# slp-rl/slamkit

Hardware: NVIDIA H100
Metric: speech-tokens/sec (SLAM seq=1024) (higher is better)
Workload: dtype bf16

## Files before the change

### include/slamkit_b200.h

```cpp
#ifndef SLAMKIT_B200_H
#define SLAMKIT_B200_H

#include <stdint.h>

#ifdef __cplusplus
extern "C" {
#endif

const char* sk_last_error(void);
int sk_version(void);
int sk_device_sm_count(void);
int sk_device_cc(void);

int sk_gemm_bf16(int M, int N, int K, const void* A, int lda, int a_mn, const void* B, int ldb, int b_mn, void* C,
                 int ldc, int out_f32, const void* bias, const void* residual, int ldr, int round_before_res, int act,
                 int force_bn, void* stream);

int sk_gemm_bf16_splitk(int M, int N, int K, const void* A, int lda, int a_mn, const void* B, int ldb, int b_mn, void* C,
                        int ldc, int accumulate, void* splitk_ws, int64_t splitk_ws_bytes, void* stream);

int sk_gemm_bf16_ws(int M, int N, int K, const void* A, int lda, int a_mn, const void* B, int ldb, int b_mn, void* C,
                    int ldc, int out_f32, const void* bias, const void* residual, int ldr, int round_before_res, int act,
                    int force_bn, void* ws, int64_t ws_bytes, void* stream);
int64_t sk_gemm_ws_bytes(void);
// ... 56 lines not shown
            int n_rot_heads, int head_dim, int inverse, int max_positions, void* stream);
int sk_swiglu_fwd(const void* gu, void* act, int M, int F, void* stream);
int sk_swiglu_bwd(const void* gu, const void* dact, void* dgu, int M, int F, void* stream);
int sk_ce_blocks(int M);
int sk_ce_fwd_bwd(const void* logits, const int64_t* labels, void* dlogits, float* partial, float* row_nll,
                  float* stats, int M, int T, int V, int ldl, float num_items, float dloss, void* stream);

int sk_attn_fwd(const void* q, const void* k, const void* v, void* o, float* lse, int B, int T, int H, int KVH, int ld,
                int ldo, int causal, float scale, void* stream);
int sk_attn_tc_fwd(const void* qkv, void* o, float* lse, int B, int T, int H, int KVH, int ld, int ldo, int causal,
                   float scale, const int32_t* seg_start, void* stream);
int sk_seg_bounds(const int32_t* pos_ids, int32_t* seg_start, int32_t* seg_end, int B, int T, void* stream);
int sk_attn_tc_bwd(const void* qkv, const void* o, const void* d_o, const float* lse, float* delta, float* partial,
                   void* dqkv, int B, int T, int H, int KVH, int ld, int ldo, int ldg, int causal, float scale,
                   const int32_t* seg_start, const int32_t* seg_end, void* stream);
int sk_attn_bwd(const void* q, const void* k, const void* v, const void* o, const void* d_o, const float* lse,
                float* delta, void* dq, void* dk, void* dv, int B, int T, int H, int KVH, int ld, int ldo, int ldg,
                int causal, float scale, void* stream);
int sk_attn_tc_fwd_split(const void* qkv_hi, const void* qkv_lo, void* o_hi, void* o_lo, int B, int T, int H, int ld,
                         int ldo, float scale, void* stream);

int sk_grad_norm(const void* grads, const int64_t* chunk_start, const int32_t* chunk_len, int n_chunks,
                 const int32_t* tensor_chunk_begin, int n_tensors, float* partial, float max_norm, int emulate_bf16,
                 float* stats, void* stream);
int sk_adamw_step(void* params, const void* grads, void* exp_avg, void* exp_avg_sq, int64_t n, float lr, float beta1,
                  float beta2, float eps, float weight_decay, int step, const float* clip_stats, void* stream);

typedef struct SkLmConfig {
  int32_t vocab_size;
  int32_t hidden;
// ... 183 lines not shown
```

### slamkit_b200/csrc/api.cu

```cuda
#include <stdlib.h>
#include "kernels.h"
#include "../../include/slamkit_b200.h"
#include <atomic>
#include <stdarg.h>
#include <stdio.h>
#include <string.h>
#include <vector>

namespace {
thread_local char g_err[1024] = "";
std::atomic<long long> g_launches{0};
}

void sk_set_error(const char* fmt, ...) {
  va_list ap;
  va_start(ap, fmt);
  vsnprintf(g_err, sizeof(g_err), fmt, ap);
  va_end(ap);
}
bool sk_pdl_enabled() {
  static const bool on = [] { const char* e = getenv("SK_PDL"); return e ? atoi(e) != 0 : true; }();
  return on;
}
void sk_count_launch() { g_launches.fetch_add(1, std::memory_order_relaxed); }
// ... 195 lines not shown
int sk_attn_tc_fwd(const void* qkv, void* o, float* lse, int B, int T, int H, int KVH, int ld, int ldo, int causal,
                   float scale, const int32_t* seg_start, void* stream) {
  SK_REQUIRE(qkv && o, "sk_attn_tc_fwd: null argument");
  return sk_attn_tc_fwd_launch(CBF(qkv), BF(o), lse, B, T, H, KVH, ld, ldo, causal, scale, S(stream), seg_start);
}
int sk_seg_bounds(const int32_t* pos_ids, int32_t* seg_start, int32_t* seg_end, int B, int T, void* stream) {
  return sk_seg_bounds_launch(pos_ids, seg_start, seg_end, B, T, S(stream));
}
int sk_attn_tc_bwd(const void* qkv, const void* o, const void* d_o, const float* lse, float* delta, float* partial,
                   void* dqkv, int B, int T, int H, int KVH, int ld, int ldo, int ldg, int causal, float scale,
                   const int32_t* seg_start, const int32_t* seg_end, void* stream) {
  SK_REQUIRE(qkv && o && d_o && lse && delta && dqkv, "sk_attn_tc_bwd: null argument");
  return sk_attn_tc_bwd_launch(CBF(qkv), CBF(o), CBF(d_o), lse, delta, partial, BF(dqkv), B, T, H, KVH, ld, ldo, ldg, causal,
                               scale, S(stream), seg_start, seg_end);
}
int sk_attn_tc_fwd_split(const void* qkv_hi, const void* qkv_lo, void* o_hi, void* o_lo, int B, int T, int H, int ld,
                         int ldo, float scale, void* stream) {
  SK_REQUIRE(qkv_hi && qkv_lo && o_hi && o_lo, "sk_attn_tc_fwd_split: null argument");
  return sk_attn_tc_fwd_split_launch(CBF(qkv_hi), CBF(qkv_lo), BF(o_hi), BF(o_lo), B, T, H, ld, ldo, scale, S(stream));
}
int sk_attn_bwd(const void* q, const void* k, const void* v, const void* o, const void* d_o, const float* lse,
                float* delta, void* dq, void* dk, void* dv, int B, int T, int H, int KVH, int ld, int ldo, int ldg,
                int causal, float scale, void* stream) {
  return sk_attn_bwd_launch(CBF(q), CBF(k), CBF(v), CBF(o), CBF(d_o), lse, delta, BF(dq), BF(dk), BF(dv), B, T, H, KVH,
                            ld, ldo, ldg, causal, scale, S(stream));
}
int sk_grad_norm(const void* grads, const int64_t* chunk_start, const int32_t* chunk_len, int n_chunks,
                 const int32_t* tensor_chunk_begin, int n_tensors, float* partial, float max_norm, int emulate_bf16,
                 float* stats, void* stream) {
  return sk_gradnorm_launch(CBF(grads), reinterpret_cast<const long*>(chunk_start), chunk_len, n_chunks,
// ... 38 lines not shown
```

### slamkit_b200/csrc/attention.cu

```cuda
#include "kernels.h"

namespace {

constexpr int HD = 64;

SK_DEVINL uint32_t tile_addr(uint32_t base, int r, int chunk) { return base + r * 128 + ((chunk ^ (r & 7)) << 4); }
SK_DEVINL uint32_t smem_base_1k(const void* p) { return (smem_u32(p) + 1023u) & ~1023u; }

SK_DEVINL void cp_async16(uint32_t saddr, const void* g, bool pred) {
  const int sz = pred ? 16 : 0;
  asm volatile("cp.async.cg.shared.global [%0], [%1], 16, %2;" ::"r"(saddr), "l"(g), "r"(sz) : "memory");
}
SK_DEVINL void cp_async_commit() { asm volatile("cp.async.commit_group;" ::: "memory"); }
template <int N>
SK_DEVINL void cp_async_wait() {
  asm volatile("cp.async.wait_group %0;" ::"n"(N) : "memory");
}

SK_DEVINL void wgmma_m64n64_rs(float (&d)[32], const uint32_t (&a)[4], uint64_t db) {
  asm volatile(
      "{\n\t.reg .pred p;\n\tsetp.eq.u32 p, 1, 1;\n\t"
      "wgmma.mma_async.sync.aligned.m64n64k16.f32.bf16.bf16 {%0,%1,%2,%3,%4,%5,%6,%7,%8,%9,%10,%11,%12,%13,%14,%15,"
      "%16,%17,%18,%19,%20,%21,%22,%23,%24,%25,%26,%27,%28,%29,%30,%31}, {%32,%33,%34,%35}, %36, p, 1, 1, 1;\n\t}\n"
      : "+f"(d[0]), "+f"(d[1]), "+f"(d[2]), "+f"(d[3]), "+f"(d[4]), "+f"(d[5]), "+f"(d[6]), "+f"(d[7]), "+f"(d[8]),
        "+f"(d[9]), "+f"(d[10]), "+f"(d[11]), "+f"(d[12]), "+f"(d[13]), "+f"(d[14]), "+f"(d[15]), "+f"(d[16]),
        "+f"(d[17]), "+f"(d[18]), "+f"(d[19]), "+f"(d[20]), "+f"(d[21]), "+f"(d[22]), "+f"(d[23]), "+f"(d[24]),
// ... 59 lines not shown
  const uint32_t sV = sK + 2 * 64 * 128;
  const int b = blockIdx.z, h = blockIdx.y;
  const int qt = gridDim.x - 1 - blockIdx.x;
  const int q0 = qt * 128;
  const int warp = threadIdx.x >> 5, lane = threadIdx.x & 31;
  const bf16* qp = q + (size_t)b * T * ld + h * HD;
  const bf16* kp = k + (size_t)b * T * ld + (h / group) * HD;
  const bf16* vp = v + (size_t)b * T * ld + (h / group) * HD;
  const float sl2 = scale * 1.4426950408889634f;

  int n_kv = (T + 63) / 64;
  if (CAUSAL) {
    const int last = min(T - 1, q0 + 127);
    n_kv = last / 64 + 1;
  }
  load_tile<128, 256>(sQ, qp, ld, q0, T);
  load_tile<64, 256>(sK, kp, ld, 0, T);
  load_tile<64, 256>(sV, vp, ld, 0, T);
  cp_async_commit();

  const uint32_t sQw = sQ + (uint32_t)(warp >> 2) * 8192u;
  float oacc[8][4];
  zero_acc(oacc);
  float m_i[2] = {-INFINITY, -INFINITY}, l_i[2] = {0.f, 0.f};
  const int row_a = q0 + warp * 16 + (lane >> 2);
  int seg_r[2] = {0, 0};
#pragma unroll
  for (int r = 0; r < 2; ++r)
    if (seg_start && row_a + 8 * r < T) seg_r[r] = seg_start[(size_t)b * T + row_a + 8 * r];

  for (int j = 0; j < n_kv; ++j) {
    const int st = j & 1;
    if (j + 1 < n_kv) {
      load_tile<64, 256>(sK + (st ^ 1) * 8192, kp, ld, (j + 1) * 64, T);
      load_tile<64, 256>(sV + (st ^ 1) * 8192, vp, ld, (j + 1) * 64, T);
      cp_async_commit();
      cp_async_wait<1>();
    } else {
      cp_async_wait<0>();
    }
    __syncthreads();

    float s[8][4];
    zero_acc(s);
    wg_a_bT(s, sQw, sK + st * 8192);

    const int k0 = j * 64;
// ... 231 lines not shown
      const float2 x = unpack_bf16(au[kq]), y = unpack_bf16(gu[kq]);
      acc += x.x * y.x + x.y * y.y;
    }
  }
  acc += __shfl_xor_sync(0xffffffffu, acc, 1);
  acc += __shfl_xor_sync(0xffffffffu, acc, 2);
  acc += __shfl_xor_sync(0xffffffffu, acc, 4);
  if (ok && (i & 7) == 0) {
    const int h = (int)(rh % H);
    const long m = rh / H;
    const long bb = m / T, t = m % T;
    delta[(bb * H + h) * T + t] = acc;
  }
}

template <bool CAUSAL>
__global__ void __launch_bounds__(128, 3)
attn_bwd_dkdv_kernel(const bf16* __restrict__ q, const bf16* __restrict__ k, const bf16* __restrict__ v,
                     const bf16* __restrict__ d_o, const float* __restrict__ lse, const float* __restrict__ delta,
                     bf16* __restrict__ dk, bf16* __restrict__ dv, int T, int ld, int ldo, int ldg, int H, int group,
                     float scale, const int* __restrict__ seg_start) {
  extern __shared__ __align__(128) uint8_t smem_attn[];
  const uint32_t sKV = smem_base_1k(smem_attn);
  const uint32_t sQ = sKV + 2 * 8192;
  const uint32_t sdO = sQ + 2 * 8192;
  float* sStat = reinterpret_cast<float*>(smem_attn + (sKV - smem_u32(smem_attn)) + 6 * 8192);
  int* sSeg = reinterpret_cast<int*>(sStat + 2 * 2 * 64);
  const int b = blockIdx.z, g = blockIdx.y;
  const int kt = blockIdx.x;
  const int k0 = kt * 64;
  const int warp = threadIdx.x >> 5, lane = threadIdx.x & 31;
  const float sl2 = scale * 1.4426950408889634f;
  const bf16* kp = k + (size_t)b * T * ld + g * HD;
  const bf16* vp = v + (size_t)b * T * ld + g * HD;

  load_tile<64, 128>(sKV, kp, ld, k0, T);
  load_tile<64, 128>(sKV + 8192, vp, ld, k0, T);
  cp_async_commit();

  const int n_qt = (T + 63) / 64;
  const int qt_begin = CAUSAL ? kt : 0;
  const int per_head = n_qt - qt_begin;
  const int n_iter = per_head * group;

  auto issue = [&](int it, int st) {
    const int h = g * group + it / per_head;
    const int qt = qt_begin + it % per_head;
    const bf16* qp = q + (size_t)b * T * ld + h * HD;
    const bf16* dop = d_o + (size_t)b * T * ldo + h * HD;
    load_tile<64, 128>(sQ + st * 8192, qp, ld, qt * 64, T);
    load_tile<64, 128>(sdO + st * 8192, dop, ldo, qt * 64, T);
    if (threadIdx.x < 64) {
      const int row = qt * 64 + threadIdx.x;
      const size_t off = ((size_t)b * H + h) * T + (row < T ? row : 0);
      sStat[(st * 2 + 0) * 64 + threadIdx.x] = row < T ? lse[off] : 0.f;
      sStat[(st * 2 + 1) * 64 + threadIdx.x] = row < T ? delta[off] : 0.f;
      sSeg[st * 64 + threadIdx.x] = (seg_start && row < T) ? seg_start[(size_t)b * T + row] : 0;
    }
    cp_async_commit();
  };
  if (n_iter > 0) issue(0, 0);

  float dkacc[8][4], dvacc[8][4];
  zero_acc(dkacc);
  zero_acc(dvacc);
  const int key_a = k0 + warp * 16 + (lane >> 2);

  for (int it = 0; it < n_iter; ++it) {
    const int st = it & 1;
    if (it + 1 < n_iter) {
      issue(it + 1, st ^ 1);
      cp_async_wait<1>();
    } else {
      cp_async_wait<0>();
    }
    __syncthreads();
    const int qt = qt_begin + it % per_head;
    const int q0 = qt * 64;
    const float* s_lse = sStat + (st * 2 + 0) * 64;
    const float* s_del = sStat + (st * 2 + 1) * 64;

    float st_acc[8][4];
    zero_acc(st_acc);
    wg_a_bT(st_acc, sKV, sQ + st * 8192);
    const int* s_seg = sSeg + st * 64;
    const bool need_mask = (CAUSAL && (q0 < k0 + 64)) || (q0 + 64 > T) || (k0 + 64 > T) || seg_start;
#pragma unroll
    for (int nt = 0; nt < 8; ++nt) {
#pragma unroll
      for (int e = 0; e < 4; ++e) {
        const int qi = nt * 8 + (lane & 3) * 2 + (e & 1);
        const int key = key_a + ((e >> 1) << 3);
        float pv = exp2f(st_acc[nt][e] * sl2 - s_lse[qi] * 1.4426950408889634f);
        if (need_mask) {
          const int qrow = q0 + qi;
          if (qrow >= T || key >= T || (CAUSAL && key > qrow) || key < s_seg[qi]) pv = 0.f;
        }
        st_acc[nt][e] = pv;
      }
    }
    uint32_t pa[4][4];
    acc_to_a(st_acc, pa);
    wg_p_b(dvacc, pa, sdO + st * 8192);

    float dp[8][4];
    zero_acc(dp);
    wg_a_bT(dp, sKV + 8192, sdO + st * 8192);
#pragma unroll
    for (int nt = 0; nt < 8; ++nt) {
#pragma unroll
      for (int e = 0; e < 4; ++e) {
        const int qi = nt * 8 + (lane & 3) * 2 + (e & 1);
        dp[nt][e] = st_acc[nt][e] * (dp[nt][e] - s_del[qi]) * scale;
      }
    }
    acc_to_a(dp, pa);
    wg_p_b(dkacc, pa, sQ + st * 8192);
    __syncthreads();
  }
#pragma unroll
  for (int r = 0; r < 2; ++r) {
    const int key = key_a + 8 * r;
    if (key < T) {
      bf16* dkp = dk + ((size_t)b * T + key) * ldg + g * HD;
      bf16* dvp = dv + ((size_t)b * T + key) * ldg + g * HD;
#pragma unroll
      for (int nt = 0; nt < 8; ++nt) {
        *reinterpret_cast<uint32_t*>(dkp + nt * 8 + (lane & 3) * 2) = pack_bf16(dkacc[nt][2 * r], dkacc[nt][2 * r + 1]);
        *reinterpret_cast<uint32_t*>(dvp + nt * 8 + (lane & 3) * 2) = pack_bf16(dvacc[nt][2 * r], dvacc[nt][2 * r + 1]);
      }
    }
  }
}

template <bool CAUSAL>
__global__ void __launch_bounds__(128)
attn_bwd_dq_kernel(const bf16* __restrict__ q, const bf16* __restrict__ k, const bf16* __restrict__ v,
                   const bf16* __restrict__ d_o, const float* __restrict__ lse, const float* __restrict__ delta,
                   bf16* __restrict__ dq, int T, int ld, int ldo, int ldg, int H, int group, float scale,
                   const int* __restrict__ seg_start) {
  extern __shared__ __align__(128) uint8_t smem_attn[];
  const uint32_t sQdO = smem_base_1k(smem_attn);
  const uint32_t sK = sQdO + 2 * 8192;
  const uint32_t sV = sK + 2 * 8192;
  const int b = blockIdx.z, h = blockIdx.y;
  const int qt = gridDim.x - 1 - blockIdx.x;
  const int q0 = qt * 64;
  const int warp = threadIdx.x >> 5, lane = threadIdx.x & 31;
  const float sl2 = scale * 1.4426950408889634f;
  const bf16* qp = q + (size_t)b * T * ld + h * HD;
  const bf16* dop = d_o + (size_t)b * T * ldo + h * HD;
  const bf16* kp = k + (size_t)b * T * ld + (h / group) * HD;
  const bf16* vp = v + (size_t)b * T * ld + (h / group) * HD;

  int n_kv = (T + 63) / 64;
  if (CAUSAL) n_kv = min(T - 1, q0 + 63) / 64 + 1;
  load_tile<64, 128>(sQdO, qp, ld, q0, T);
  load_tile<64, 128>(sQdO + 8192, dop, ldo, q0, T);
  load_tile<64, 128>(sK, kp, ld, 0, T);
  load_tile<64, 128>(sV, vp, ld, 0, T);
  cp_async_commit();

  const int row_a = q0 + warp * 16 + (lane >> 2);
  float lse_r[2], del_r[2];
  int seg_r[2];
#pragma unroll
  for (int r = 0; r < 2; ++r) {
    const int row = row_a + 8 * r;
    const size_t off = ((size_t)b * H + h) * T + (row < T ? row : 0);
    lse_r[r] = row < T ? lse[off] * 1.4426950408889634f : 0.f;
    del_r[r] = row < T ? delta[off] : 0.f;
    seg_r[r] = (seg_start && row < T) ? seg_start[(size_t)b * T + row] : 0;
  }
  float dqacc[8][4];
  zero_acc(dqacc);

  for (int j = 0; j < n_kv; ++j) {
    const int st = j & 1;
    if (j + 1 < n_kv) {
      load_tile<64, 128>(sK + (st ^ 1) * 8192, kp, ld, (j + 1) * 64, T);
      load_tile<64, 128>(sV + (st ^ 1) * 8192, vp, ld, (j + 1) * 64, T);
      cp_async_commit();
      cp_async_wait<1>();
    } else {
      cp_async_wait<0>();
    }
    __syncthreads();
    const int k0 = j * 64;
    float s[8][4];
    zero_acc(s);
    wg_a_bT(s, sQdO, sK + st * 8192);
    const bool need_mask = (CAUSAL && (k0 + 63 > q0 + warp * 16)) || (k0 + 64 > T) || (q0 + 64 > T) || seg_start;
#pragma unroll
    for (int nt = 0; nt < 8; ++nt) {
#pragma unroll
      for (int e = 0; e < 4; ++e) {
        float pv = exp2f(s[nt][e] * sl2 - lse_r[e >> 1]);
        if (need_mask) {
          const int key = k0 + nt * 8 + (lane & 3) * 2 + (e & 1);
          const int row = row_a + ((e >> 1) << 3);
          if (row >= T || key >= T || (CAUSAL && key > row) || key < seg_r[e >> 1]) pv = 0.f;
        }
        s[nt][e] = pv;
      }
    }
    float dp[8][4];
    zero_acc(dp);
    wg_a_bT(dp, sQdO + 8192, sV + st * 8192);
#pragma unroll
    for (int nt = 0; nt < 8; ++nt) {
#pragma unroll
      for (int e = 0; e < 4; ++e) dp[nt][e] = s[nt][e] * (dp[nt][e] - del_r[e >> 1]) * scale;
    }
    uint32_t pa[4][4];
    acc_to_a(dp, pa);
    wg_p_b(dqacc, pa, sK + st * 8192);
    __syncthreads();
  }
#pragma unroll
  for (int r = 0; r < 2; ++r) {
    const int row = row_a + 8 * r;
    if (row < T) {
      bf16* dqp = dq + ((size_t)b * T + row) * ldg + h * HD;
#pragma unroll
      for (int nt = 0; nt < 8; ++nt)
        *reinterpret_cast<uint32_t*>(dqp + nt * 8 + (lane & 3) * 2) = pack_bf16(dqacc[nt][2 * r], dqacc[nt][2 * r + 1]);
    }
  }
}

constexpr int FWD_SMEM = 128 * 128 + 4 * 8192 + 1024;
constexpr int DKDV_SMEM = 6 * 8192 + 2 * 2 * 64 * 4 + 2 * 64 * 4 + 1024;
constexpr int DQ_SMEM = 6 * 8192 + 1024;
constexpr int FWD_SPLIT_SMEM = 2 * 128 * 128 + 8 * 8192 + 1024;

template <typename K>
int set_smem(K kernel, int bytes) {
  SK_CUDA_CHECK(cudaFuncSetAttribute(kernel, cudaFuncAttributeMaxDynamicSharedMemorySize, bytes));
  return 0;
}

}

int sk_attn_fwd_launch(const bf16* q, const bf16* k, const bf16* v, bf16* o, float* lse, int B, int T, int H, int KVH,
                       int ld, int ldo, int causal, float scale, cudaStream_t s, const int* seg_start) {
  SK_REQUIRE(seg_start == nullptr || causal, "attention: document segments need the causal kernel");
  SK_REQUIRE(B > 0 && T > 0 && H > 0 && KVH > 0, "attention: bad shape B=%d T=%d H=%d KVH=%d", B, T, H, KVH);
  SK_REQUIRE(H % KVH == 0, "attention: H must be a multiple of KVH");
  SK_REQUIRE(ld % 8 == 0 && ldo % 8 == 0, "attention: leading dims must be multiples of 8");
  static bool init = false;
  if (!init) {
    if (set_smem(attn_fwd_kernel<true>, FWD_SMEM)) return -2;
    if (set_smem(attn_fwd_kernel<false>, FWD_SMEM)) return -2;
    init = true;
  }
  dim3 grid((T + 127) / 128, H, B);
  sk_prof_begin(1, s);
  if (causal) attn_fwd_kernel<true><<<grid, 256, FWD_SMEM, s>>>(q, k, v, o, lse, T, ld, ldo, H, H / KVH, scale, seg_start);
  else attn_fwd_kernel<false><<<grid, 256, FWD_SMEM, s>>>(q, k, v, o, lse, T, ld, ldo, H, H / KVH, scale, nullptr);
  sk_prof_end(s);
  SK_LAUNCH_CHECK();
  return 0;
}

int sk_attn_bwd_launch(const bf16* q, const bf16* k, const bf16* v, const bf16* o, const bf16* d_o, const float* lse,
                       float* delta, bf16* dq, bf16* dk, bf16* dv, int B, int T, int H, int KVH, int ld, int ldo,
                       int ldg, int causal, float scale, cudaStream_t s, const int* seg_start) {
  SK_REQUIRE(seg_start == nullptr || causal, "attention: document segments need the causal kernels");
  SK_REQUIRE(B > 0 && T > 0 && H > 0 && KVH > 0, "attention: bad shape B=%d T=%d H=%d KVH=%d", B, T, H, KVH);
  SK_REQUIRE(H % KVH == 0, "attention: H must be a multiple of KVH");
  SK_REQUIRE(ld % 8 == 0 && ldo % 8 == 0 && ldg % 2 == 0, "attention: ld and ldo must be multiples of 8 and ldg even");
  static bool init = false;
  if (!init) {
    if (set_smem(attn_bwd_dkdv_kernel<true>, DKDV_SMEM)) return -2;
    if (set_smem(attn_bwd_dkdv_kernel<false>, DKDV_SMEM)) return -2;
    if (set_smem(attn_bwd_dq_kernel<true>, DQ_SMEM)) return -2;
    if (set_smem(attn_bwd_dq_kernel<false>, DQ_SMEM)) return -2;
    init = true;
  }
  const long total = (long)B * T * H * 8;
  sk_prof_begin(1, s);
  SK_CUDA_CHECK(sk_launch_pdl(attn_delta_kernel, dim3((int)((total + 255) / 256)), dim3(256), (size_t)(0), s, o, d_o, delta, B, T, H, ldo));
  SK_LAUNCH_CHECK();
  const int group = H / KVH;
  dim3 g1((T + 63) / 64, KVH, B), g2((T + 63) / 64, H, B);
  if (causal) {
    attn_bwd_dkdv_kernel<true><<<g1, 128, DKDV_SMEM, s>>>(q, k, v, d_o, lse, delta, dk, dv, T, ld, ldo, ldg, H, group, scale,
                                                          seg_start);
    SK_LAUNCH_CHECK();
    attn_bwd_dq_kernel<true><<<g2, 128, DQ_SMEM, s>>>(q, k, v, d_o, lse, delta, dq, T, ld, ldo, ldg, H, group, scale, seg_start);
  } else {
    attn_bwd_dkdv_kernel<false><<<g1, 128, DKDV_SMEM, s>>>(q, k, v, d_o, lse, delta, dk, dv, T, ld, ldo, ldg, H, group, scale,
                                                           nullptr);
    SK_LAUNCH_CHECK();
    attn_bwd_dq_kernel<false><<<g2, 128, DQ_SMEM, s>>>(q, k, v, d_o, lse, delta, dq, T, ld, ldo, ldg, H, group, scale, nullptr);
  }
  sk_prof_end(s);
  SK_LAUNCH_CHECK();
  return 0;
}

int sk_attn_fwd_split_launch(const bf16* q_hi, const bf16* q_lo, const bf16* k_hi, const bf16* k_lo, const bf16* v_hi,
                             const bf16* v_lo, bf16* o_hi, bf16* o_lo, int B, int T, int H, int ld, int ldo, float scale,
                             cudaStream_t s) {
  SK_REQUIRE(B > 0 && T > 0 && H > 0, "attention: bad shape B=%d T=%d H=%d", B, T, H);
  SK_REQUIRE(ld % 8 == 0 && ldo % 8 == 0, "attention: leading dims must be multiples of 8");
  static bool init = false;
  if (!init) {
    if (set_smem(attn_fwd_split_kernel, FWD_SPLIT_SMEM)) return -2;
    init = true;
  }
// ... 15 lines not shown
}

int sk_attn_tc_fwd_launch(const bf16* qkv, bf16* o, float* lse, int B, int T, int H, int KVH, int ld, int ldo, int causal,
                          float scale, cudaStream_t s, const int* seg_start) {
  return sk_attn_fwd_launch(qkv, qkv + H * HD, qkv + (H + KVH) * HD, o, lse, B, T, H, KVH, ld, ldo, causal, scale, s,
                            seg_start);
}

int sk_attn_tc_bwd_launch(const bf16* qkv, const bf16* o, const bf16* d_o, const float* lse, float* delta, float* partial,
                          bf16* dqkv, int B, int T, int H, int KVH, int ld, int ldo, int ldg, int causal, float scale,
                          cudaStream_t s, const int* seg_start, const int* seg_end, const bf16* rope_cos,
                          const bf16* rope_sin, const int* pos_ids, int max_pos) {
  (void)partial;
  SK_REQUIRE((seg_start == nullptr) == (seg_end == nullptr), "attn_tc_bwd: seg_start and seg_end go together");
  SK_REQUIRE((rope_cos == nullptr) == (rope_sin == nullptr) && (rope_cos == nullptr || max_pos > 0), "attn_tc_bwd: rope tables go together");
  int rc = sk_attn_bwd_launch(qkv, qkv + H * HD, qkv + (H + KVH) * HD, o, d_o, lse, delta, dqkv, dqkv + H * HD,
                              dqkv + (H + KVH) * HD, B, T, H, KVH, ld, ldo, ldg, causal, scale, s, seg_start);
  if (rc) return rc;
  if (rope_cos) return sk_rope_launch(dqkv, rope_cos, rope_sin, pos_ids, B * T, T, ldg, H + KVH, HD, 1, max_pos, s);
  return 0;
}

int sk_attn_tc_fwd_split_launch(const bf16* qkv_hi, const bf16* qkv_lo, bf16* o_hi, bf16* o_lo, int B, int T, int H, int ld,
                                int ldo, float scale, cudaStream_t s) {
  return sk_attn_fwd_split_launch(qkv_hi, qkv_lo, qkv_hi + H * HD, qkv_lo + H * HD, qkv_hi + 2 * H * HD, qkv_lo + 2 * H * HD,
                                  o_hi, o_lo, B, T, H, ld, ldo, scale, s);
}
```

### slamkit_b200/csrc/kernels.h

```cpp
#pragma once
#include "common.cuh"

int sk_make_tmap_2d(CUtensorMap* out, const void* ptr, int elem_bytes, uint64_t inner, uint64_t outer, uint64_t ld,
                    uint32_t box_inner, uint32_t box_outer);
int sk_make_tmap_3d(CUtensorMap* out, const void* ptr, uint64_t inner, uint64_t rows, uint64_t batch, uint64_t row_stride,
                    uint64_t batch_stride, uint32_t box_rows);
int sk_pick_bn(int M, int N, int force_bn, bool fit_forced, bool fit, bool whole_heads);
size_t sk_gemm_ws_min_bytes(void);
struct SkGemmEx {
  int M, N, K;
  int batch;
  int a_mode;
  int passes;
  const void *A, *A_lo;
  int lda, a_mn;
  long a_inner, a_rows, a_row_stride, a_batch_stride;
  const void *B, *B_lo;
  int ldb, b_mn;
  void *C, *C_lo;
  int ldc, out_f32;
  const void* bias;
  int bias_f32;
  const void *residual, *residual_lo;
  int ldr, round_before_res, act;
// ... 56 lines not shown
                            float eps, cudaStream_t s);
extern "C" int sk_layernorm_bwd_blocks(void);
int sk_layernorm_bwd_launch(const bf16* dy, const bf16* x, const bf16* w, const float* mean, const float* rstd, const bf16* dres,
                            bf16* dx, bf16* dw, bf16* db, float* dw_partial, float* db_partial, int M, int D, int accumulate,
                            cudaStream_t s);
int sk_opt_embed_fwd_launch(const int64_t* ids, const int32_t* pos_ids, const bf16* E, const bf16* P, bf16* out, int M, int T, int D,
                            int V, int n_pos, cudaStream_t s);
int sk_opt_pos_bwd_launch(const int32_t* pos_ids, const bf16* dx, float* scratch, bf16* dP, int M, int T, int D, int n_pos,
                          int accumulate, cudaStream_t s);
int sk_relu_bwd_launch(bf16* g, const bf16* a, long n, cudaStream_t s);

int sk_attn_fwd_launch(const bf16* q, const bf16* k, const bf16* v, bf16* o, float* lse, int B, int T, int H, int KVH,
                       int ld, int ldo, int causal, float scale, cudaStream_t s, const int* seg_start = nullptr);
int sk_attn_bwd_launch(const bf16* q, const bf16* k, const bf16* v, const bf16* o, const bf16* d_o, const float* lse,
                       float* delta, bf16* dq, bf16* dk, bf16* dv, int B, int T, int H, int KVH, int ld, int ldo,
                       int ldg, int causal, float scale, cudaStream_t s, const int* seg_start = nullptr);
int sk_attn_fwd_split_launch(const bf16* q_hi, const bf16* q_lo, const bf16* k_hi, const bf16* k_lo, const bf16* v_hi,
                             const bf16* v_lo, bf16* o_hi, bf16* o_lo, int B, int T, int H, int ld, int ldo, float scale,
                             cudaStream_t s);

int sk_attn_tc_fwd_split_launch(const bf16* qkv_hi, const bf16* qkv_lo, bf16* o_hi, bf16* o_lo, int B, int T, int H, int ld,
                                int ldo, float scale, cudaStream_t s);
int sk_attn_tc_bwd_launch(const bf16* qkv, const bf16* o, const bf16* d_o, const float* lse, float* delta, float* partial,
                          bf16* dqkv, int B, int T, int H, int KVH, int ld, int ldo, int ldg, int causal, float scale,
                          cudaStream_t s, const int* seg_start = nullptr, const int* seg_end = nullptr,
                          const bf16* rope_cos = nullptr, const bf16* rope_sin = nullptr, const int* pos_ids = nullptr,
                          int max_pos = 0);
int sk_attn_tc_fwd_launch(const bf16* qkv, bf16* o, float* lse, int B, int T, int H, int KVH, int ld, int ldo, int causal,
                          float scale, cudaStream_t s, const int* seg_start = nullptr);

int sk_kv_prefill_launch(const bf16* qkv, long layer_stride, int ldq, bf16* cache, const int32_t* lens, int L, int B, int T,
// ... 42 lines not shown
```

### slamkit_b200/ops.py

```python
from __future__ import annotations

import ctypes as C
from typing import Optional, Tuple

import torch

from . import _lib as L


def _bf16(t: torch.Tensor) -> torch.Tensor:
    assert t.is_cuda and t.dtype == torch.bfloat16, "expected a CUDA bf16 tensor"
    return t


_gemm_ws = {}


def gemm_workspace(device) -> torch.Tensor:
    lib = L.require_cuda()
    key = torch.device(device).index or 0
    if key not in _gemm_ws:
        _gemm_ws[key] = torch.zeros(int(lib.sk_gemm_ws_bytes()) + (64 << 20), dtype=torch.uint8, device=device)
    return _gemm_ws[key]

# ... 219 lines not shown
    L.check(lib.sk_seg_bounds(L.ptr(pos), L.ptr(ss), L.ptr(se), B, T, L.stream_ptr()))
    return ss, se


def attn_tc_fwd(qkv: torch.Tensor, B: int, T: int, H: int, KVH: int, causal: bool, scale: float,
                seg_start: Optional[torch.Tensor] = None):
    lib = L.require_cuda()
    o = torch.empty((B * T, H * 64), device=qkv.device, dtype=torch.bfloat16)
    lse = torch.empty((B, H, T), device=qkv.device, dtype=torch.float32)
    L.check(lib.sk_attn_tc_fwd(L.ptr(qkv), L.ptr(o), L.ptr(lse), B, T, H, KVH, qkv.stride(0), o.stride(0), int(causal),
                               L.f32(scale), L.ptr(seg_start), L.stream_ptr()))
    return o, lse


def attn_tc_bwd(qkv, o, d_o, lse, B, T, H, KVH, causal: bool, scale: float, seg_start: Optional[torch.Tensor] = None,
                seg_end: Optional[torch.Tensor] = None) -> torch.Tensor:
    lib = L.require_cuda()
    dqkv = torch.empty_like(qkv)
    delta = torch.empty_like(lse)
    L.check(lib.sk_attn_tc_bwd(L.ptr(qkv), L.ptr(o), L.ptr(d_o), L.ptr(lse), L.ptr(delta), L.ptr(None), L.ptr(dqkv),
                               B, T, H, KVH, qkv.stride(0), o.stride(0), dqkv.stride(0), int(causal), L.f32(scale),
                               L.ptr(seg_start), L.ptr(seg_end), L.stream_ptr()))
    return dqkv


def attn_tc_fwd_split(qkv_hi: torch.Tensor, qkv_lo: torch.Tensor, B: int, T: int, H: int, scale: float):
    lib = L.require_cuda()
    assert qkv_hi.stride(0) == qkv_lo.stride(0)
    o_hi = torch.empty((B * T, H * 64), device=qkv_hi.device, dtype=torch.bfloat16)
    o_lo = torch.empty_like(o_hi)
    L.check(lib.sk_attn_tc_fwd_split(L.ptr(qkv_hi), L.ptr(qkv_lo), L.ptr(o_hi), L.ptr(o_lo), B, T, H, qkv_hi.stride(0),
                                     o_hi.stride(0), L.f32(scale), L.stream_ptr()))
    return o_hi, o_lo

# ... 19 lines not shown
```

Baseline: 153,400.

## Fuse attention backward into one PDL kernel with RoPE epilogue and segment skipping

Merges the dK/dV and dQ backward kernels into a single launch indexed by a unit id, launched with programmatic dependent launch, and folds the inverse RoPE into the gradient store instead of a separate rope pass. It also deepens the dK/dV pipeline to three stages with async cp of the lse/delta/segment stats, issues the S and dP wgmmas asynchronously so they overlap, and skips KV/Q tiles outside the document segment in forward and backward. The fused kernel shares one smem size and a launch bound across both unit types, which may hurt occupancy for the dQ path. Inverse RoPE now rounds inside the epilogue, which may change numerics slightly.

```diff
diff --git a/include/slamkit_b200.h b/include/slamkit_b200.h
--- a/include/slamkit_b200.h
+++ b/include/slamkit_b200.h
@@ -94,6 +94,10 @@
 int sk_attn_tc_bwd(const void* qkv, const void* o, const void* d_o, const float* lse, float* delta, float* partial,
                    void* dqkv, int B, int T, int H, int KVH, int ld, int ldo, int ldg, int causal, float scale,
                    const int32_t* seg_start, const int32_t* seg_end, void* stream);
+int sk_attn_tc_bwd_rope(const void* qkv, const void* o, const void* d_o, const float* lse, float* delta, void* dqkv, int B,
+                        int T, int H, int KVH, int ld, int ldo, int ldg, int causal, float scale, const int32_t* seg_start,
+                        const int32_t* seg_end, const void* rope_cos, const void* rope_sin, const int32_t* pos_ids,
+                        int max_positions, void* stream);
 int sk_attn_bwd(const void* q, const void* k, const void* v, const void* o, const void* d_o, const float* lse,
                 float* delta, void* dq, void* dk, void* dv, int B, int T, int H, int KVH, int ld, int ldo, int ldg,
                 int causal, float scale, void* stream);
diff --git a/slamkit_b200/csrc/api.cu b/slamkit_b200/csrc/api.cu
--- a/slamkit_b200/csrc/api.cu
+++ b/slamkit_b200/csrc/api.cu
@@ -233,6 +233,14 @@
   return sk_attn_tc_bwd_launch(CBF(qkv), CBF(o), CBF(d_o), lse, delta, partial, BF(dqkv), B, T, H, KVH, ld, ldo, ldg, causal,
                                scale, S(stream), seg_start, seg_end);
 }
+int sk_attn_tc_bwd_rope(const void* qkv, const void* o, const void* d_o, const float* lse, float* delta, void* dqkv, int B,
+                        int T, int H, int KVH, int ld, int ldo, int ldg, int causal, float scale, const int32_t* seg_start,
+                        const int32_t* seg_end, const void* rope_cos, const void* rope_sin, const int32_t* pos_ids,
+                        int max_positions, void* stream) {
+  SK_REQUIRE(qkv && o && d_o && lse && delta && dqkv && rope_cos && rope_sin, "sk_attn_tc_bwd_rope: null argument");
+  return sk_attn_tc_bwd_launch(CBF(qkv), CBF(o), CBF(d_o), lse, delta, nullptr, BF(dqkv), B, T, H, KVH, ld, ldo, ldg, causal,
+                               scale, S(stream), seg_start, seg_end, CBF(rope_cos), CBF(rope_sin), pos_ids, max_positions);
+}
 int sk_attn_tc_fwd_split(const void* qkv_hi, const void* qkv_lo, void* o_hi, void* o_lo, int B, int T, int H, int ld,
                          int ldo, float scale, void* stream) {
   SK_REQUIRE(qkv_hi && qkv_lo && o_hi && o_lo, "sk_attn_tc_fwd_split: null argument");
diff --git a/slamkit_b200/csrc/attention.cu b/slamkit_b200/csrc/attention.cu
--- a/slamkit_b200/csrc/attention.cu
+++ b/slamkit_b200/csrc/attention.cu
@@ -10,6 +10,10 @@
 SK_DEVINL void cp_async16(uint32_t saddr, const void* g, bool pred) {
   const int sz = pred ? 16 : 0;
   asm volatile("cp.async.cg.shared.global [%0], [%1], 16, %2;" ::"r"(saddr), "l"(g), "r"(sz) : "memory");
+}
+SK_DEVINL void cp_async4(uint32_t saddr, const void* g, bool pred) {
+  const int sz = pred ? 4 : 0;
+  asm volatile("cp.async.ca.shared.global [%0], [%1], 4, %2;" ::"r"(saddr), "l"(g), "r"(sz) : "memory");
 }
 SK_DEVINL void cp_async_commit() { asm volatile("cp.async.commit_group;" ::: "memory"); }
 template <int N>
@@ -99,9 +103,12 @@
     const int last = min(T - 1, q0 + 127);
     n_kv = last / 64 + 1;
   }
+  griddep_launch();
+  griddep_wait();
+  const int j0 = seg_start ? seg_start[(size_t)b * T + q0] / 64 : 0;
   load_tile<128, 256>(sQ, qp, ld, q0, T);
-  load_tile<64, 256>(sK, kp, ld, 0, T);
-  load_tile<64, 256>(sV, vp, ld, 0, T);
+  load_tile<64, 256>(sK, kp, ld, j0 * 64, T);
+  load_tile<64, 256>(sV, vp, ld, j0 * 64, T);
   cp_async_commit();
 
   const uint32_t sQw = sQ + (uint32_t)(warp >> 2) * 8192u;
@@ -114,8 +121,8 @@
   for (int r = 0; r < 2; ++r)
     if (seg_start && row_a + 8 * r < T) seg_r[r] = seg_start[(size_t)b * T + row_a + 8 * r];
 
-  for (int j = 0; j < n_kv; ++j) {
-    const int st = j & 1;
+  for (int j = j0; j < n_kv; ++j) {
+    const int st = (j - j0) & 1;
     if (j + 1 < n_kv) {
       load_tile<64, 256>(sK + (st ^ 1) * 8192, kp, ld, (j + 1) * 64, T);
       load_tile<64, 256>(sV + (st ^ 1) * 8192, vp, ld, (j + 1) * 64, T);
@@ -377,25 +384,97 @@
   }
 }
 
+constexpr int DKDV_STAGES = 3;
+
+struct BwdArgs {
+  const bf16 *q, *k, *v, *d_o;
+  const float *lse, *delta;
+  bf16 *dq, *dk, *dv;
+  int B, T, ld, ldo, ldg, H, KVH, group;
+  float scale;
+  const int* seg_start;
+  const bf16 *rope_cos, *rope_sin;
+  const int* pos_ids;
+  int max_pos;
+  int n_dkdv;
+};
+
+template <int ACC>
+SK_DEVINL void wgmma_m64n64_ss(float (&d)[32], uint64_t da, uint64_t db) {
+  if constexpr (ACC == 0) {
+    asm volatile(
+        "{\n\t.reg .pred p;\n\tsetp.ne.u32 p, 0, 0;\n\t"
+        "wgmma.mma_async.sync.aligned.m64n64k16.f32.bf16.bf16 {%0,%1,%2,%3,%4,%5,%6,%7,%8,%9,%10,%11,%12,%13,%14,%15,"
+        "%16,%17,%18,%19,%20,%21,%22,%23,%24,%25,%26,%27,%28,%29,%30,%31}, %32, %33, p, 1, 1, 0, 0;\n\t}\n"
+        : "=f"(d[0]), "=f"(d[1]), "=f"(d[2]), "=f"(d[3]), "=f"(d[4]), "=f"(d[5]), "=f"(d[6]), "=f"(d[7]), "=f"(d[8]),
+          "=f"(d[9]), "=f"(d[10]), "=f"(d[11]), "=f"(d[12]), "=f"(d[13]), "=f"(d[14]), "=f"(d[15]), "=f"(d[16]),
+          "=f"(d[17]), "=f"(d[18]), "=f"(d[19]), "=f"(d[20]), "=f"(d[21]), "=f"(d[22]), "=f"(d[23]), "=f"(d[24]),
+          "=f"(d[25]), "=f"(d[26]), "=f"(d[27]), "=f"(d[28]), "=f"(d[29]), "=f"(d[30]), "=f"(d[31])
+        : "l"(da), "l"(db));
+  } else {
+    wgmma_m64n64<0, 0>(d, da, db);
+  }
+}
+
+SK_DEVINL void wg_a_bT_async(float (&acc)[8][4], uint32_t sA, uint32_t sB) {
+  float(&d)[32] = reinterpret_cast<float(&)[32]>(acc);
+  wgmma_fence();
+  wgmma_m64n64_ss<0>(d, gmma_desc_sw128(sA, 16, 1024), gmma_desc_sw128(sB, 16, 1024));
+#pragma unroll
+  for (int ks = 1; ks < 4; ++ks)
+    wgmma_m64n64_ss<1>(d, gmma_desc_sw128(sA + ks * 32, 16, 1024), gmma_desc_sw128(sB + ks * 32, 16, 1024));
+  wgmma_commit();
+}
+SK_DEVINL void wg_p_b_async(float (&acc)[8][4], const uint32_t (&p)[4][4], uint32_t sB) {
+  float(&d)[32] = reinterpret_cast<float(&)[32]>(acc);
+  wgmma_fence();
+#pragma unroll
+  for (int kk = 0; kk < 4; ++kk) wgmma_m64n64_rs(d, p[kk], gmma_desc_sw128(sB + kk * 2048, 8192, 1024));
+  wgmma_commit();
+}
+
+SK_DEVINL void store_grad_row(bf16* dst, const float (&acc)[8][4], int r, int lane, const BwdArgs& a, size_t m) {
+  if (!a.rope_cos) {
+#pragma unroll
+    for (int nt = 0; nt < 8; ++nt)
+      *reinterpret_cast<uint32_t*>(dst + nt * 8 + (lane & 3) * 2) = pack_bf16(acc[nt][2 * r], acc[nt][2 * r + 1]);
+    return;
+  }
+  int pos = a.pos_ids ? a.pos_ids[m] : (int)(m % a.T);
+  pos = max(0, min(pos, a.max_pos - 1));
+#pragma unroll
+  for (int nt = 0; nt < 4; ++nt) {
+    const int c = nt * 8 + (lane & 3) * 2;
+    const float2 x1 = unpack_bf16(pack_bf16(acc[nt][2 * r], acc[nt][2 * r + 1]));
+    const float2 x2 = unpack_bf16(pack_bf16(acc[nt + 4][2 * r], acc[nt + 4][2 * r + 1]));
+    const float2 cs = unpack_bf16(__ldg(reinterpret_cast<const unsigned int*>(a.rope_cos + (size_t)pos * 32 + c)));
+    float2 sn = unpack_bf16(__ldg(reinterpret_cast<const unsigned int*>(a.rope_sin + (size_t)pos * 32 + c)));
+    sn.x = -sn.x;
+    sn.y = -sn.y;
+    *reinterpret_cast<uint32_t*>(dst + c) =
+        pack_bf16(bf16_round(x1.x * cs.x) + bf16_round(-x2.x * sn.x), bf16_round(x1.y * cs.y) + bf16_round(-x2.y * sn.y));
+    *reinterpret_cast<uint32_t*>(dst + c + 32) =
+        pack_bf16(bf16_round(x2.x * cs.x) + bf16_round(x1.x * sn.x), bf16_round(x2.y * cs.y) + bf16_round(x1.y * sn.y));
+  }
+}
+
 template <bool CAUSAL>
-__global__ void __launch_bounds__(128, 3)
-attn_bwd_dkdv_kernel(const bf16* __restrict__ q, const bf16* __restrict__ k, const bf16* __restrict__ v,
-                     const bf16* __restrict__ d_o, const float* __restrict__ lse, const float* __restrict__ delta,
-                     bf16* __restrict__ dk, bf16* __restrict__ dv, int T, int ld, int ldo, int ldg, int H, int group,
-                     float scale, const int* __restrict__ seg_start) {
-  extern __shared__ __align__(128) uint8_t smem_attn[];
+SK_DEVINL void bwd_dkdv_unit(const BwdArgs& a, uint8_t* smem_attn, int kt, int g, int b) {
   const uint32_t sKV = smem_base_1k(smem_attn);
   const uint32_t sQ = sKV + 2 * 8192;
-  const uint32_t sdO = sQ + 2 * 8192;
-  float* sStat = reinterpret_cast<float*>(smem_attn + (sKV - smem_u32(smem_attn)) + 6 * 8192);
-  int* sSeg = reinterpret_cast<int*>(sStat + 2 * 2 * 64);
-  const int b = blockIdx.z, g = blockIdx.y;
-  const int kt = blockIdx.x;
+  const uint32_t sdO = sQ + DKDV_STAGES * 8192;
+  const uint32_t sStat = sdO + DKDV_STAGES * 8192;
+  const uint32_t sSeg = sStat + DKDV_STAGES * 2 * 64 * 4;
+  const float* stat_p = reinterpret_cast<const float*>(smem_attn + (sStat - smem_u32(smem_attn)));
+  const int* seg_p = reinterpret_cast<const int*>(smem_attn + (sSeg - smem_u32(smem_attn)));
+  const int T = a.T, ld = a.ld, ldo = a.ldo, H = a.H, group = a.group;
+  const float scale = a.scale;
+  const int* seg_start = a.seg_start;
   const int k0 = kt * 64;
   const int warp = threadIdx.x >> 5, lane = threadIdx.x & 31;
   const float sl2 = scale * 1.4426950408889634f;
-  const bf16* kp = k + (size_t)b * T * ld + g * HD;
-  const bf16* vp = v + (size_t)b * T * ld + g * HD;
+  const bf16* kp = a.k + (size_t)b * T * ld + g * HD;
+  const bf16* vp = a.v + (size_t)b * T * ld + g * HD;
 
   load_tile<64, 128>(sKV, kp, ld, k0, T);
   load_tile<64, 128>(sKV + 8192, vp, ld, k0, T);
@@ -403,26 +482,38 @@
 
   const int n_qt = (T + 63) / 64;
   const int qt_begin = CAUSAL ? kt : 0;
-  const int per_head = n_qt - qt_begin;
+  int qt_end = n_qt;
+  if (seg_start) {
+    int lo = qt_begin, hi = n_qt;
+    while (lo < hi) {
+      const int mid = (lo + hi) >> 1;
+      if (seg_start[(size_t)b * T + mid * 64] > k0 + 63) hi = mid;
+      else lo = mid + 1;
+    }
+    qt_end = lo;
+  }
+  const int per_head = qt_end - qt_begin;
   const int n_iter = per_head * group;
 
   auto issue = [&](int it, int st) {
     const int h = g * group + it / per_head;
     const int qt = qt_begin + it % per_head;
-    const bf16* qp = q + (size_t)b * T * ld + h * HD;
-    const bf16* dop = d_o + (size_t)b * T * ldo + h * HD;
+    const bf16* qp = a.q + (size_t)b * T * ld + h * HD;
+    const bf16* dop = a.d_o + (size_t)b * T * ldo + h * HD;
     load_tile<64, 128>(sQ + st * 8192, qp, ld, qt * 64, T);
     load_tile<64, 128>(sdO + st * 8192, dop, ldo, qt * 64, T);
     if (threadIdx.x < 64) {
       const int row = qt * 64 + threadIdx.x;
-      const size_t off = ((size_t)b * H + h) * T + (row < T ? row : 0);
-      sStat[(st * 2 + 0) * 64 + threadIdx.x] = row < T ? lse[off] : 0.f;
-      sStat[(st * 2 + 1) * 64 + threadIdx.x] = row < T ? delta[off] : 0.f;
-      sSeg[st * 64 + threadIdx.x] = (seg_start && row < T) ? seg_start[(size_t)b * T + row] : 0;
+      const bool ok = row < T;
+      const size_t off = ((size_t)b * H + h) * T + (ok ? row : 0);
+      cp_async4(sStat + ((st * 2 + 0) * 64 + threadIdx.x) * 4, a.lse + off, ok);
+      cp_async4(sStat + ((st * 2 + 1) * 64 + threadIdx.x) * 4, a.delta + off, ok);
+      const void* seg_src = seg_start ? static_cast<const void*>(seg_start + (size_t)b * T + (ok ? row : 0)) : a.lse;
+      cp_async4(sSeg + (st * 64 + threadIdx.x) * 4, seg_src, ok && seg_start);
     }
     cp_async_commit();
   };
-  if (n_iter > 0) issue(0, 0);
+  for (int i = 0; i < DKDV_STAGES - 1 && i < n_iter; ++i) issue(i, i);
 
   float dkacc[8][4], dvacc[8][4];
   zero_acc(dkacc);
@@ -430,9 +521,11 @@
   const int key_a = k0 + warp * 16 + (lane >> 2);
 
   for (int it = 0; it < n_iter; ++it) {
-    const int st = it & 1;
-    if (it + 1 < n_iter) {
-      issue(it + 1, st ^ 1);
+    const int st = it % DKDV_STAGES;
+    if (it + 2 < n_iter) {
+      issue(it + 2, (it + 2) % DKDV_STAGES);
+      cp_async_wait<2>();
+    } else if (it + 1 < n_iter) {
       cp_async_wait<1>();
     } else {
       cp_async_wait<0>();
@@ -440,13 +533,14 @@
     __syncthreads();
     const int qt = qt_begin + it % per_head;
     const int q0 = qt * 64;
-    const float* s_lse = sStat + (st * 2 + 0) * 64;
-    const float* s_del = sStat + (st * 2 + 1) * 64;
-
-    float st_acc[8][4];
-    zero_acc(st_acc);
-    wg_a_bT(st_acc, sKV, sQ + st * 8192);
-    const int* s_seg = sSeg + st * 64;
+    const float* s_lse = stat_p + (st * 2 + 0) * 64;
+    const float* s_del = stat_p + (st * 2 + 1) * 64;
+
+    float st_acc[8][4], dp[8][4];
+    wg_a_bT_async(st_acc, sKV, sQ + st * 8192);
+    wg_a_bT_async(dp, sKV + 8192, sdO + st * 8192);
+    wgmma_wait<1>();
+    const int* s_seg = seg_p + st * 64;
     const bool need_mask = (CAUSAL && (q0 < k0 + 64)) || (q0 + 64 > T) || (k0 + 64 > T) || seg_start;
 #pragma unroll
     for (int nt = 0; nt < 8; ++nt) {
@@ -464,11 +558,8 @@
     }
     uint32_t pa[4][4];
     acc_to_a(st_acc, pa);
-    wg_p_b(dvacc, pa, sdO + st * 8192);
-
-    float dp[8][4];
-    zero_acc(dp);
-    wg_a_bT(dp, sKV + 8192, sdO + st * 8192);
+    wg_p_b_async(dvacc, pa, sdO + st * 8192);
+    wgmma_wait<1>();
 #pragma unroll
     for (int nt = 0; nt < 8; ++nt) {
 #pragma unroll
@@ -477,51 +568,49 @@
         dp[nt][e] = st_acc[nt][e] * (dp[nt][e] - s_del[qi]) * scale;
       }
     }
+    wgmma_wait<0>();
     acc_to_a(dp, pa);
-    wg_p_b(dkacc, pa, sQ + st * 8192);
+    wg_p_b_async(dkacc, pa, sQ + st * 8192);
+    wgmma_wait<0>();
     __syncthreads();
   }
 #pragma unroll
   for (int r = 0; r < 2; ++r) {
     const int key = key_a + 8 * r;
     if (key < T) {
-      bf16* dkp = dk + ((size_t)b * T + key) * ldg + g * HD;
-      bf16* dvp = dv + ((size_t)b * T + key) * ldg + g * HD;
-#pragma unroll
-      for (int nt = 0; nt < 8; ++nt) {
-        *reinterpret_cast<uint32_t*>(dkp + nt * 8 + (lane & 3) * 2) = pack_bf16(dkacc[nt][2 * r], dkacc[nt][2 * r + 1]);
+      const size_t m = (size_t)b * T + key;
+      store_grad_row(a.dk + m * a.ldg + g * HD, dkacc, r, lane, a, m);
+      bf16* dvp = a.dv + m * a.ldg + g * HD;
+#pragma unroll
+      for (int nt = 0; nt < 8; ++nt)
         *reinterpret_cast<uint32_t*>(dvp + nt * 8 + (lane & 3) * 2) = pack_bf16(dvacc[nt][2 * r], dvacc[nt][2 * r + 1]);
-      }
     }
   }
 }
 
 template <bool CAUSAL>
-__global__ void __launch_bounds__(128)
-attn_bwd_dq_kernel(const bf16* __restrict__ q, const bf16* __restrict__ k, const bf16* __restrict__ v,
-                   const bf16* __restrict__ d_o, const float* __restrict__ lse, const float* __restrict__ delta,
-                   bf16* __restrict__ dq, int T, int ld, int ldo, int ldg, int H, int group, float scale,
-                   const int* __restrict__ seg_start) {
-  extern __shared__ __align__(128) uint8_t smem_attn[];
+SK_DEVINL void bwd_dq_unit(const BwdArgs& a, uint8_t* smem_attn, int qt, int h, int b) {
   const uint32_t sQdO = smem_base_1k(smem_attn);
   const uint32_t sK = sQdO + 2 * 8192;
   const uint32_t sV = sK + 2 * 8192;
-  const int b = blockIdx.z, h = blockIdx.y;
-  const int qt = gridDim.x - 1 - blockIdx.x;
+  const int T = a.T, ld = a.ld, H = a.H, group = a.group;
+  const float scale = a.scale;
+  const int* seg_start = a.seg_start;
   const int q0 = qt * 64;
   const int warp = threadIdx.x >> 5, lane = threadIdx.x & 31;
   const float sl2 = scale * 1.4426950408889634f;
-  const bf16* qp = q + (size_t)b * T * ld + h * HD;
-  const bf16* dop = d_o + (size_t)b * T * ldo + h * HD;
-  const bf16* kp = k + (size_t)b * T * ld + (h / group) * HD;
-  const bf16* vp = v + (size_t)b * T * ld + (h / group) * HD;
+  const bf16* qp = a.q + (size_t)b * T * ld + h * HD;
+  const bf16* dop = a.d_o + (size_t)b * T * a.ldo + h * HD;
+  const bf16* kp = a.k + (size_t)b * T * ld + (h / group) * HD;
+  const bf16* vp = a.v + (size_t)b * T * ld + (h / group) * HD;
 
   int n_kv = (T + 63) / 64;
   if (CAUSAL) n_kv = min(T - 1, q0 + 63) / 64 + 1;
+  const int j0 = seg_start ? seg_start[(size_t)b * T + q0] / 64 : 0;
   load_tile<64, 128>(sQdO, qp, ld, q0, T);
-  load_tile<64, 128>(sQdO + 8192, dop, ldo, q0, T);
-  load_tile<64, 128>(sK, kp, ld, 0, T);
-  load_tile<64, 128>(sV, vp, ld, 0, T);
+  load_tile<64, 128>(sQdO + 8192, dop, a.ldo, q0, T);
+  load_tile<64, 128>(sK, kp, ld, j0 * 64, T);
+  load_tile<64, 128>(sV, vp, ld, j0 * 64, T);
   cp_async_commit();
 
   const int row_a = q0 + warp * 16 + (lane >> 2);
@@ -531,15 +620,15 @@
   for (int r = 0; r < 2; ++r) {
     const int row = row_a + 8 * r;
     const size_t off = ((size_t)b * H + h) * T + (row < T ? row : 0);
-    lse_r[r] = row < T ? lse[off] * 1.4426950408889634f : 0.f;
-    del_r[r] = row < T ? delta[off] : 0.f;
+    lse_r[r] = row < T ? a.lse[off] * 1.4426950408889634f : 0.f;
+    del_r[r] = row < T ? a.delta[off] : 0.f;
     seg_r[r] = (seg_start && row < T) ? seg_start[(size_t)b * T + row] : 0;
   }
   float dqacc[8][4];
   zero_acc(dqacc);
 
-  for (int j = 0; j < n_kv; ++j) {
-    const int st = j & 1;
+  for (int j = j0; j < n_kv; ++j) {
+    const int st = (j - j0) & 1;
     if (j + 1 < n_kv) {
       load_tile<64, 128>(sK + (st ^ 1) * 8192, kp, ld, (j + 1) * 64, T);
       load_tile<64, 128>(sV + (st ^ 1) * 8192, vp, ld, (j + 1) * 64, T);
@@ -550,9 +639,10 @@
     }
     __syncthreads();
     const int k0 = j * 64;
-    float s[8][4];
-    zero_acc(s);
-    wg_a_bT(s, sQdO, sK + st * 8192);
+    float s[8][4], dp[8][4];
+    wg_a_bT_async(s, sQdO, sK + st * 8192);
+    wg_a_bT_async(dp, sQdO + 8192, sV + st * 8192);
+    wgmma_wait<1>();
     const bool need_mask = (CAUSAL && (k0 + 63 > q0 + warp * 16)) || (k0 + 64 > T) || (q0 + 64 > T) || seg_start;
 #pragma unroll
     for (int nt = 0; nt < 8; ++nt) {
@@ -567,9 +657,7 @@
         s[nt][e] = pv;
       }
     }
-    float dp[8][4];
-    zero_acc(dp);
-    wg_a_bT(dp, sQdO + 8192, sV + st * 8192);
+    wgmma_wait<0>();
 #pragma unroll
     for (int nt = 0; nt < 8; ++nt) {
 #pragma unroll
@@ -577,24 +665,38 @@
     }
     uint32_t pa[4][4];
     acc_to_a(dp, pa);
-    wg_p_b(dqacc, pa, sK + st * 8192);
+    wg_p_b_async(dqacc, pa, sK + st * 8192);
+    wgmma_wait<0>();
     __syncthreads();
   }
 #pragma unroll
   for (int r = 0; r < 2; ++r) {
     const int row = row_a + 8 * r;
     if (row < T) {
-      bf16* dqp = dq + ((size_t)b * T + row) * ldg + h * HD;
-#pragma unroll
-      for (int nt = 0; nt < 8; ++nt)
-        *reinterpret_cast<uint32_t*>(dqp + nt * 8 + (lane & 3) * 2) = pack_bf16(dqacc[nt][2 * r], dqacc[nt][2 * r + 1]);
-    }
+      const size_t m = (size_t)b * T + row;
+      store_grad_row(a.dq + m * a.ldg + h * HD, dqacc, r, lane, a, m);
+    }
+  }
+}
+
+template <bool CAUSAL>
+__global__ void __launch_bounds__(128, 3) attn_bwd_kernel(const BwdArgs a) {
+  extern __shared__ __align__(128) uint8_t smem_attn[];
+  griddep_launch();
+  griddep_wait();
+  const int u = blockIdx.x;
+  if (u < a.n_dkdv) {
+    const int kt = u / (a.KVH * a.B), r = u % (a.KVH * a.B);
+    bwd_dkdv_unit<CAUSAL>(a, smem_attn, kt, r % a.KVH, r / a.KVH);
+  } else {
+    const int v = u - a.n_dkdv, n_qt = (a.T + 63) / 64;
+    const int qt = n_qt - 1 - v / (a.H * a.B), r = v % (a.H * a.B);
+    bwd_dq_unit<CAUSAL>(a, smem_attn, qt, r % a.H, r / a.H);
   }
 }
 
 constexpr int FWD_SMEM = 128 * 128 + 4 * 8192 + 1024;
-constexpr int DKDV_SMEM = 6 * 8192 + 2 * 2 * 64 * 4 + 2 * 64 * 4 + 1024;
-constexpr int DQ_SMEM = 6 * 8192 + 1024;
+constexpr int BWD_SMEM = (2 + 2 * DKDV_STAGES) * 8192 + DKDV_STAGES * 3 * 64 * 4 + 1024;
 constexpr int FWD_SPLIT_SMEM = 2 * 128 * 128 + 8 * 8192 + 1024;
 
 template <typename K>
@@ -619,8 +721,8 @@
   }
   dim3 grid((T + 127) / 128, H, B);
   sk_prof_begin(1, s);
-  if (causal) attn_fwd_kernel<true><<<grid, 256, FWD_SMEM, s>>>(q, k, v, o, lse, T, ld, ldo, H, H / KVH, scale, seg_start);
-  else attn_fwd_kernel<false><<<grid, 256, FWD_SMEM, s>>>(q, k, v, o, lse, T, ld, ldo, H, H / KVH, scale, nullptr);
+  SK_CUDA_CHECK(sk_launch_pdl(causal ? attn_fwd_kernel<true> : attn_fwd_kernel<false>, grid, dim3(256), (size_t)FWD_SMEM, s,
+                              q, k, v, o, lse, T, ld, ldo, H, H / KVH, scale, causal ? seg_start : nullptr));
   sk_prof_end(s);
   SK_LAUNCH_CHECK();
   return 0;
@@ -628,36 +730,27 @@
 
 int sk_attn_bwd_launch(const bf16* q, const bf16* k, const bf16* v, const bf16* o, const bf16* d_o, const float* lse,
                        float* delta, bf16* dq, bf16* dk, bf16* dv, int B, int T, int H, int KVH, int ld, int ldo,
-                       int ldg, int causal, float scale, cudaStream_t s, const int* seg_start) {
+                       int ldg, int causal, float scale, cudaStream_t s, const int* seg_start, const bf16* rope_cos,
+                       const bf16* rope_sin, const int* pos_ids, int max_pos) {
   SK_REQUIRE(seg_start == nullptr || causal, "attention: document segments need the causal kernels");
   SK_REQUIRE(B > 0 && T > 0 && H > 0 && KVH > 0, "attention: bad shape B=%d T=%d H=%d KVH=%d", B, T, H, KVH);
   SK_REQUIRE(H % KVH == 0, "attention: H must be a multiple of KVH");
   SK_REQUIRE(ld % 8 == 0 && ldo % 8 == 0 && ldg % 2 == 0, "attention: ld and ldo must be multiples of 8 and ldg even");
   static bool init = false;
   if (!init) {
-    if (set_smem(attn_bwd_dkdv_kernel<true>, DKDV_SMEM)) return -2;
-    if (set_smem(attn_bwd_dkdv_kernel<false>, DKDV_SMEM)) return -2;
-    if (set_smem(attn_bwd_dq_kernel<true>, DQ_SMEM)) return -2;
-    if (set_smem(attn_bwd_dq_kernel<false>, DQ_SMEM)) return -2;
+    if (set_smem(attn_bwd_kernel<true>, BWD_SMEM)) return -2;
+    if (set_smem(attn_bwd_kernel<false>, BWD_SMEM)) return -2;
     init = true;
   }
   const long total = (long)B * T * H * 8;
   sk_prof_begin(1, s);
   SK_CUDA_CHECK(sk_launch_pdl(attn_delta_kernel, dim3((int)((total + 255) / 256)), dim3(256), (size_t)(0), s, o, d_o, delta, B, T, H, ldo));
   SK_LAUNCH_CHECK();
-  const int group = H / KVH;
-  dim3 g1((T + 63) / 64, KVH, B), g2((T + 63) / 64, H, B);
-  if (causal) {
-    attn_bwd_dkdv_kernel<true><<<g1, 128, DKDV_SMEM, s>>>(q, k, v, d_o, lse, delta, dk, dv, T, ld, ldo, ldg, H, group, scale,
-                                                          seg_start);
-    SK_LAUNCH_CHECK();
-    attn_bwd_dq_kernel<true><<<g2, 128, DQ_SMEM, s>>>(q, k, v, d_o, lse, delta, dq, T, ld, ldo, ldg, H, group, scale, seg_start);
-  } else {
-    attn_bwd_dkdv_kernel<false><<<g1, 128, DKDV_SMEM, s>>>(q, k, v, d_o, lse, delta, dk, dv, T, ld, ldo, ldg, H, group, scale,
-                                                           nullptr);
-    SK_LAUNCH_CHECK();
-    attn_bwd_dq_kernel<false><<<g2, 128, DQ_SMEM, s>>>(q, k, v, d_o, lse, delta, dq, T, ld, ldo, ldg, H, group, scale, nullptr);
-  }
+  const int n_t = (T + 63) / 64;
+  const BwdArgs a{q, k, v, d_o, lse, delta, dq, dk, dv, B, T, ld, ldo, ldg, H, KVH, H / KVH, scale,
+                  causal ? seg_start : nullptr, rope_cos, rope_sin, pos_ids, max_pos, n_t * KVH * B};
+  SK_CUDA_CHECK(sk_launch_pdl(causal ? attn_bwd_kernel<true> : attn_bwd_kernel<false>, dim3(n_t * (KVH + H) * B), dim3(128),
+                              (size_t)BWD_SMEM, s, a));
   sk_prof_end(s);
   SK_LAUNCH_CHECK();
   return 0;
@@ -703,11 +796,11 @@
   (void)partial;
   SK_REQUIRE((seg_start == nullptr) == (seg_end == nullptr), "attn_tc_bwd: seg_start and seg_end go together");
   SK_REQUIRE((rope_cos == nullptr) == (rope_sin == nullptr) && (rope_cos == nullptr || max_pos > 0), "attn_tc_bwd: rope tables go together");
-  int rc = sk_attn_bwd_launch(qkv, qkv + H * HD, qkv + (H + KVH) * HD, o, d_o, lse, delta, dqkv, dqkv + H * HD,
-                              dqkv + (H + KVH) * HD, B, T, H, KVH, ld, ldo, ldg, causal, scale, s, seg_start);
-  if (rc) return rc;
-  if (rope_cos) return sk_rope_launch(dqkv, rope_cos, rope_sin, pos_ids, B * T, T, ldg, H + KVH, HD, 1, max_pos, s);
-  return 0;
+  SK_REQUIRE(rope_cos == nullptr || pos_ids != nullptr || T <= max_pos, "attn_tc_bwd: rope table rows (%d) do not cover T=%d",
+             max_pos, T);
+  return sk_attn_bwd_launch(qkv, qkv + H * HD, qkv + (H + KVH) * HD, o, d_o, lse, delta, dqkv, dqkv + H * HD,
+                            dqkv + (H + KVH) * HD, B, T, H, KVH, ld, ldo, ldg, causal, scale, s, seg_start, rope_cos,
+                            rope_sin, pos_ids, max_pos);
 }
 
 int sk_attn_tc_fwd_split_launch(const bf16* qkv_hi, const bf16* qkv_lo, bf16* o_hi, bf16* o_lo, int B, int T, int H, int ld,
diff --git a/slamkit_b200/csrc/kernels.h b/slamkit_b200/csrc/kernels.h
--- a/slamkit_b200/csrc/kernels.h
+++ b/slamkit_b200/csrc/kernels.h
@@ -94,7 +94,9 @@
                        int ld, int ldo, int causal, float scale, cudaStream_t s, const int* seg_start = nullptr);
 int sk_attn_bwd_launch(const bf16* q, const bf16* k, const bf16* v, const bf16* o, const bf16* d_o, const float* lse,
                        float* delta, bf16* dq, bf16* dk, bf16* dv, int B, int T, int H, int KVH, int ld, int ldo,
-                       int ldg, int causal, float scale, cudaStream_t s, const int* seg_start = nullptr);
+                       int ldg, int causal, float scale, cudaStream_t s, const int* seg_start = nullptr,
+                       const bf16* rope_cos = nullptr, const bf16* rope_sin = nullptr, const int* pos_ids = nullptr,
+                       int max_pos = 0);
 int sk_attn_fwd_split_launch(const bf16* q_hi, const bf16* q_lo, const bf16* k_hi, const bf16* k_lo, const bf16* v_hi,
                              const bf16* v_lo, bf16* o_hi, bf16* o_lo, int B, int T, int H, int ld, int ldo, float scale,
                              cudaStream_t s);
diff --git a/slamkit_b200/ops.py b/slamkit_b200/ops.py
--- a/slamkit_b200/ops.py
+++ b/slamkit_b200/ops.py
@@ -257,10 +257,17 @@
 
 
 def attn_tc_bwd(qkv, o, d_o, lse, B, T, H, KVH, causal: bool, scale: float, seg_start: Optional[torch.Tensor] = None,
-                seg_end: Optional[torch.Tensor] = None) -> torch.Tensor:
+                seg_end: Optional[torch.Tensor] = None, rope_cos: Optional[torch.Tensor] = None,
+                rope_sin: Optional[torch.Tensor] = None, pos_ids: Optional[torch.Tensor] = None) -> torch.Tensor:
     lib = L.require_cuda()
     dqkv = torch.empty_like(qkv)
     delta = torch.empty_like(lse)
+    if rope_cos is not None:
+        L.check(lib.sk_attn_tc_bwd_rope(L.ptr(qkv), L.ptr(o), L.ptr(d_o), L.ptr(lse), L.ptr(delta), L.ptr(dqkv), B, T, H,
+                                        KVH, qkv.stride(0), o.stride(0), dqkv.stride(0), int(causal), L.f32(scale),
+                                        L.ptr(seg_start), L.ptr(seg_end), L.ptr(rope_cos), L.ptr(rope_sin),
+                                        L.ptr(pos_ids), rope_cos.shape[0], L.stream_ptr()))
+        return dqkv
     L.check(lib.sk_attn_tc_bwd(L.ptr(qkv), L.ptr(o), L.ptr(d_o), L.ptr(lse), L.ptr(delta), L.ptr(None), L.ptr(dqkv),
                                B, T, H, KVH, qkv.stride(0), o.stride(0), dqkv.stride(0), int(causal), L.f32(scale),
                                L.ptr(seg_start), L.ptr(seg_end), L.stream_ptr()))
```

Measured after the change: 156,900 (median of 6 runs). 2.3% higher.
